# ethz-asl/laser_slam

Measured on AMD Instinct MI355X. Metric: scans_per_sec, higher is better.
Workload: dtype f32

## Files before the change

### laser_slam_amd/csrc/lsgpu_cone.hip.h

```cpp
#pragma once
#include "lsgpu_knn.hip.h"

namespace lsgpu {

constexpr int kConeGF4 = 3;
constexpr int kConePad = 16;
constexpr uint32_t kConeMaxWin = 512;

struct ConeDev {
  float ox, oy, oz;
  float z0, rs;
  float cs;
  int rows, cols;
  const float4* soa;
  const uint32_t* map;
  const uint32_t* tab;
  const float4* rowz;
};

__device__ __forceinline__ void cone_dir(float vx, float vy, float vz, float& inv_rho, float& zeta, float& pa, float& rxy,
                                         float& inv_h) {
  const float r2 = __fmaf_rn(vy, vy, vx * vx);
  inv_rho = __builtin_amdgcn_rsqf(__fmaf_rn(vz, vz, r2));
  rxy = __builtin_amdgcn_sqrtf(r2);
  zeta = vz * inv_rho;
  inv_h = __builtin_amdgcn_rcpf(fabsf(vx) + fabsf(vy));
  const float t = vy * inv_h;
  pa = vx >= 0.f ? (vy >= 0.f ? t : 4.f + t) : 2.f - t;
}

__device__ __forceinline__ uint32_t cone_clampu(float t, int hi) {
  return (uint32_t)fminf(fmaxf(t, 0.f), (float)hi);
}

__global__ __launch_bounds__(256) void k_cone_keys(const float4* __restrict__ pts, int64_t n, ConeDev c,
                                                   uint64_t* __restrict__ keys, uint32_t* __restrict__ vals) {
  const int64_t i = (int64_t)blockIdx.x * 256 + threadIdx.x;
  if (i >= n) return;
  const float4 p = pts[i];
  float inv_rho, zeta, pa, rxy, inv_h;
  cone_dir(p.x - c.ox, p.y - c.oy, p.z - c.oz, inv_rho, zeta, pa, rxy, inv_h);
  if (!(fabsf(zeta) <= 1.5f)) zeta = 0.f;
  if (!(pa >= 0.f && pa <= 4.f)) pa = 0.f;
  const uint32_t row = cone_clampu(floorf((zeta - c.z0) * c.rs), c.rows - 1);
  const uint32_t col = cone_clampu(floorf(pa * c.cs), c.cols - 1);
  keys[i] = (uint64_t)row * (uint32_t)c.cols + col;
  vals[i] = (uint32_t)i;
}

__global__ __launch_bounds__(256) void k_cone_gather(const float4* __restrict__ pts, const uint32_t* __restrict__ perm,
                                                     const uint64_t* __restrict__ keys, int64_t n, ConeDev c,
                                                     float* __restrict__ soa, uint32_t* __restrict__ map,
                                                     uint32_t* __restrict__ tab) {
  const int64_t j = (int64_t)blockIdx.x * 256 + threadIdx.x;
  const int lane = threadIdx.x & 63;
  const int64_t npad = ((n + 3) & ~(int64_t)3) + kConePad;
  const uint32_t nkeys = (uint32_t)c.rows * (uint32_t)c.cols;
  uint32_t gap_lo = 0, gap_hi = 0;
  uint32_t pos = 0;
  const bool valid = j < n;
  if (valid) {
    const uint32_t i = perm[j];
    const float4 p = pts[i];
    float* g = soa + 4 * kConeGF4 * (j >> 2) + (j & 3);
    g[0] = p.x; g[4] = p.y; g[8] = p.z; map[j] = i;
    const uint32_t key = (uint32_t)keys[j];
    gap_lo = j > 0 ? (uint32_t)keys[j - 1] + 1u : 0u;
    gap_hi = key + 1u;
    pos = (uint32_t)j;
  } else if (j < npad) {
    float* g = soa + 4 * kConeGF4 * (j >> 2) + (j & 3);
    g[0] = kPadCoord; g[4] = kPadCoord; g[8] = kPadCoord; map[j] = 0u;
    if (j == n) { gap_lo = (uint32_t)keys[n - 1] + 1u; gap_hi = nkeys + 1u; pos = (uint32_t)n; }
  }
  const uint32_t glen = gap_hi - gap_lo;
  if (glen >= 1u && glen <= 6u) {
    tab[gap_lo] = pos;
    for (uint32_t k = 1u; k < glen; ++k) tab[gap_lo + k] = pos;
// ... 431 lines not shown
```

### laser_slam_amd/csrc/lsgpu_grid.hip.h

```cpp
#pragma once
#include "lsgpu_common.hip.h"

namespace lsgpu {

struct RefStats {
  double sum[3];
  float mn[3];
  float mx[3];
  float zmn, zmx;
};

__global__ __launch_bounds__(256) void k_ref_stats(const float4* __restrict__ in, int64_t n,
                                                   RefStats* __restrict__ partials) {
  double sx = 0, sy = 0, sz = 0;
  float mnx = INFINITY, mny = INFINITY, mnz = INFINITY, mxx = -INFINITY, mxy = -INFINITY,
        mxz = -INFINITY, zmn = INFINITY, zmx = -INFINITY;
  for (int64_t i = (int64_t)blockIdx.x * 256 + threadIdx.x; i < n; i += (int64_t)gridDim.x * 256) {
    const float4 p = in[i];
    sx += p.x; sy += p.y; sz += p.z;
    mnx = fminf(mnx, p.x); mny = fminf(mny, p.y); mnz = fminf(mnz, p.z);
    mxx = fmaxf(mxx, p.x); mxy = fmaxf(mxy, p.y); mxz = fmaxf(mxz, p.z);
    const float r2 = p.x * p.x + p.y * p.y + p.z * p.z;
    if (r2 > 0.f) {
      const float zeta = p.z * __builtin_amdgcn_rsqf(r2);
// ... 68 lines not shown
      gm.mean[d] = (float)(r.sum[d] / (double)n);
      mn[d] = r.mn[d] - gm.mean[d];
      mx[d] = r.mx[d] - gm.mean[d];
      if (!isfinite(mn[d]) || !isfinite(mx[d])) gm.bad = 1;
    }
    const float ext = fmaxf(fmaxf(mx[0] - mn[0], mx[1] - mn[1]), mx[2] - mn[2]);
    int bits = 11, fine = 5;
    float h0 = cell_size_cfg > 0.f ? cell_size_cfg : 0.125f;
    while (bits < 13 && h0 * (float)((1 << bits) - 1) < ext * 1.0001f) { ++bits; --fine; }
    while (!gm.bad && h0 * (float)((1 << bits) - 1) < ext * 1.0001f) h0 *= 2.f;
    gm.ox = mn[0]; gm.oy = mn[1]; gm.oz = mn[2];
    gm.h0 = h0; gm.hf = h0 / (float)(1 << fine); gm.inv_hf = 1.0f / gm.hf; gm.fine = fine; gm.bits = bits;
    gm.zeta_lo = r.zmn; gm.zeta_hi = r.zmx;
    gm.origin_inside = 1;
    for (int d = 0; d < 3; ++d) {
      const float m = 0.1f * (r.mx[d] - r.mn[d]) + 1e-3f;
      if (!(r.mn[d] - m <= 0.f && 0.f <= r.mx[d] + m)) gm.origin_inside = 0;
    }
    if (!(r.zmn <= r.zmx)) gm.origin_inside = 0;
    *geom = gm;
  }
}

__global__ __launch_bounds__(256) void k_ref_keys(const float4* __restrict__ in, int64_t n,
                                                  const GeomDev* __restrict__ geom,
                                                  uint64_t* __restrict__ keys,
                                                  uint32_t* __restrict__ vals) {
  const int64_t i = (int64_t)blockIdx.x * 256 + threadIdx.x;
  if (i >= n) return;
  const GeomDev g = *geom;
  const float mx = g.mean[0], my = g.mean[1], mz = g.mean[2];
  const float4 p = in[i];
  const int lim = (1 << (g.bits + g.fine)) - 1;
  const int ix = fine_coord(p.x - mx, g.ox, g.inv_hf, lim);
  const int iy = fine_coord(p.y - my, g.oy, g.inv_hf, lim);
  const int iz = fine_coord(p.z - mz, g.oz, g.inv_hf, lim);
  keys[i] = morton3((uint32_t)ix, (uint32_t)iy, (uint32_t)iz);
  vals[i] = (uint32_t)i;
}

constexpr int kAngElev = 1024, kAngSect = 4096;

__device__ __forceinline__ void angular_cell(const float4& p, float inv_elev, float inv_sect, uint32_t& eb,
                                             uint32_t& sec, float& azim, float& range) {
  const float rho = sqrtf(p.x * p.x + p.y * p.y);
  const float elev = atan2f(p.z, rho);
  azim = atan2f(p.y, p.x) + 3.1415927f;
  range = sqrtf(rho * rho + p.z * p.z);
  eb = (uint32_t)fminf(fmaxf((elev + 1.5707964f) * inv_elev, 0.f), (float)(kAngElev - 1));
  sec = (uint32_t)fminf(fmaxf(azim * inv_sect, 0.f), (float)(kAngSect - 1));
}

constexpr int kDecElev = 181, kDecSect = 361, kDecCells = 65536;
__global__ __launch_bounds__(256) void k_query_ang_hist(const float4* __restrict__ in, int64_t n,
                                                        uint32_t* __restrict__ cells) {
  const int64_t i = (int64_t)blockIdx.x * 256 + threadIdx.x;
  uint32_t cell = 0xFFFFFFFFu;
  if (i < n) {
    const float4 p = in[i];
    const float elev = atan2f(p.z, sqrtf(p.x * p.x + p.y * p.y)), azim = atan2f(p.y, p.x) + 3.1415927f;
    const uint32_t eb = (uint32_t)fminf(fmaxf((elev + 1.5707964f) * 57.29578f, 0.f), (float)(kDecElev - 1));
    const uint32_t sec = (uint32_t)fminf(fmaxf(azim * 57.29578f, 0.f), (float)(kDecSect - 1));
    cell = ((eb * kDecSect + sec) * 40503u) & 0xFFFFu;
  }
  const int lane = threadIdx.x & 63;
  const uint32_t prev = (uint32_t)__shfl_up((int)cell, 1, 64);
  const bool head = lane == 0 || cell != prev;
  const unsigned long long heads = __ballot(head);
  if (head && cell != 0xFFFFFFFFu) {
    const unsigned long long later = lane == 63 ? 0ull : (heads >> (lane + 1));
    const int run = later ? __ffsll((long long)later) : 64 - lane;
    atomicAdd(&cells[cell], (uint32_t)run);
  }
}

__global__ __launch_bounds__(1024) void k_query_order(uint32_t* __restrict__ cells, int forced, float elev_deg,
                                                      float sect_deg) {
  __shared__ uint32_t occ[16], tot[16];
  uint32_t o = 0, t = 0;
  for (int i = threadIdx.x; i < kDecCells; i += 1024) { const uint32_t c = cells[i]; o += c ? 1u : 0u; t += c; }
  o = wave_sum_u32(o); t = wave_sum_u32(t);
  if ((threadIdx.x & 63) == 0) { occ[threadIdx.x >> 6] = o; tot[threadIdx.x >> 6] = t; }
  __syncthreads();
  if (threadIdx.x == 0) {
    o = 0; t = 0;
    for (int w = 0; w < 16; ++w) { o += occ[w]; t += tot[w]; }
    uint32_t* out = cells + kDecCells;
    out[0] = o; out[1] = t;
    const float m = o ? (float)t / (float)o : 54.f;
    const float f = sqrtf(54.f / fmaxf(m, 1.f));
    const float e = elev_deg > 0.f ? elev_deg : fminf(fmaxf(0.8f * f, 0.2f), 4.f);
    const float sc = sect_deg > 0.f ? sect_deg : fminf(fmaxf(0.35f * f, 0.1f), 2.f);
    const uint32_t automatic = (o < 64u && t > 4096u) ? 0u : 1u;
    out[2] = forced >= 0 ? (uint32_t)forced : automatic;
    out[3] = __float_as_uint(57.29578f / e);
    out[4] = __float_as_uint(57.29578f / sc);
  }
}

__global__ __launch_bounds__(256) void k_query_keys(const float4* __restrict__ in, int64_t n,
                                                    uint64_t* __restrict__ keys,
                                                    uint32_t* __restrict__ vals, const uint32_t* __restrict__ order_flag) {
  const int64_t i = (int64_t)blockIdx.x * 256 + threadIdx.x;
  if (i >= n) return;
  const float4 p = in[i];
  if (*order_flag == 1u) {
    uint32_t e32, s32; float azim, range;
    angular_cell(p, __uint_as_float(order_flag[1]), __uint_as_float(order_flag[2]), e32, s32, azim, range);
    const uint64_t eb = e32, sec = s32;
    const uint64_t rb = (uint64_t)fminf(fmaxf(range, 0.f), 1023.f);
    const uint64_t fine = (uint64_t)fminf(fmaxf(azim * 10430.378f, 0.f), 65535.f);
    keys[i] = (((eb * 4096ull + sec) * 1024ull + rb) << 16) | fine;
    vals[i] = (uint32_t)i;
    return;
  }
  const float lim = 65535.f, half = 32768.f;
  const uint32_t ix = (uint32_t)fminf(fmaxf(floorf(p.x * 128.f) + half, 0.f), lim);
  const uint32_t iy = (uint32_t)fminf(fmaxf(floorf(p.y * 128.f) + half, 0.f), lim);
  const uint32_t iz = (uint32_t)fminf(fmaxf(floorf(p.z * 128.f) + half, 0.f), lim);
  keys[i] = morton3(ix, iy, iz);
  vals[i] = (uint32_t)i;
}

__global__ __launch_bounds__(256) void k_ref_gather(const float4* __restrict__ in,
                                                    const float* __restrict__ nrm_in, int64_t n,
                                                    const uint32_t* __restrict__ perm,
                                                    const GeomDev* __restrict__ geom, float4* __restrict__ pts,
                                                    float4* __restrict__ nrm,
                                                    uint32_t* __restrict__ inv) {
  const float mx = geom->mean[0], my = geom->mean[1], mz = geom->mean[2];
  const int64_t j = (int64_t)blockIdx.x * 256 + threadIdx.x;
  if (j >= n) {
    if (j < n + 8) pts[j] = make_float4(3e18f, 3e18f, 3e18f, 0.f);
    return;
  }
  const uint32_t s = perm[j];
  const float4 p = in[s];
  pts[j] = make_float4(p.x - mx, p.y - my, p.z - mz, __uint_as_float(s));
  float4 nn = make_float4(0.f, 0.f, 0.f, 0.f);
  if (nrm_in) { nn.x = nrm_in[3 * (int64_t)s]; nn.y = nrm_in[3 * (int64_t)s + 1]; nn.z = nrm_in[3 * (int64_t)s + 2]; }
  nrm[j] = nn;
  inv[s] = (uint32_t)j;
}

// ... 7 lines not shown
  const float3 q = xform(T, p.x, p.y, p.z);
  out[j] = make_float4(q.x, q.y, q.z, __uint_as_float(s));
}

__global__ __launch_bounds__(256) void k_transform(const float4* __restrict__ in, int64_t n,
                                                   Mat34 T, float4* __restrict__ out) {
  const int64_t i = (int64_t)blockIdx.x * 256 + threadIdx.x;
  if (i >= n) return;
  const float4 p = in[i];
  const float3 q = xform(T, p.x, p.y, p.z);
  out[i] = make_float4(q.x, q.y, q.z, p.w);
}

__global__ __launch_bounds__(256) void k_rotate3(const float* __restrict__ in, int64_t n, Mat34 T, float* __restrict__ out) {
  const int64_t i = (int64_t)blockIdx.x * 256 + threadIdx.x;
  if (i >= n) return;
  const float x = in[3 * i], y = in[3 * i + 1], z = in[3 * i + 2];
  out[3 * i + 0] = __fmaf_rn(T.m[2], z, __fmaf_rn(T.m[1], y, T.m[0] * x));
  out[3 * i + 1] = __fmaf_rn(T.m[6], z, __fmaf_rn(T.m[5], y, T.m[4] * x));
  out[3 * i + 2] = __fmaf_rn(T.m[10], z, __fmaf_rn(T.m[9], y, T.m[8] * x));
}

__global__ __launch_bounds__(256) void k_chunk_flags(const uint64_t* __restrict__ keys, int64_t n,
                                                     const GeomDev* __restrict__ geom, uint32_t* __restrict__ flags) {
  const int64_t i = (int64_t)blockIdx.x * 256 + threadIdx.x;
  if (i >= n) return;
  const int fine = geom->fine;
  uint32_t f = ((i & (kChunkMax - 1)) == 0);
  if (i > 0 && ((keys[i] ^ keys[i - 1]) >> (3 * fine)) != 0) f = 1;
  flags[i] = f;
}

__global__ __launch_bounds__(256) void k_chunk_bounds(const uint32_t* __restrict__ flags,
                                                      const uint32_t* __restrict__ cidx, int64_t n,
                                                      uint32_t* __restrict__ bounds) {
  const int64_t i = (int64_t)blockIdx.x * 256 + threadIdx.x;
  if (i >= n) return;
  if (flags[i]) bounds[cidx[i] - 1] = (uint32_t)i;
  if (i == n - 1) bounds[cidx[i]] = (uint32_t)n;
}

__global__ __launch_bounds__(256) void k_chunk_boxes(const float4* __restrict__ pts,
                                                     const uint32_t* __restrict__ bounds,
                                                     uint32_t nchunks,
                                                     ChunkDesc* __restrict__ chunks) {
  const uint32_t c = blockIdx.x * 4u + (threadIdx.x >> 6);
  if (c >= nchunks) return;
  const int lane = threadIdx.x & 63;
// ... 132 lines not shown
```

### laser_slam_amd/csrc/lsgpu_icp.hip

```cpp
#include <cstring>
#include <cmath>
#include <cstdio>
#include <cstdlib>
#include <string>
#include <vector>
#include <chrono>
#include <functional>
#include <system_error>
#include <thread>
#include <utility>

#include <dlfcn.h>

#include <hip/hip_runtime.h>
#include <rccl/rccl.h>

#include "../../include/lsgpu_icp.h"
#include "lsgpu_grid.hip.h"
#include "lsgpu_tuning.h"
#include "lsgpu_policy.h"
#include "lsgpu_knn.hip.h"
#include "lsgpu_knn_k.hip.h"
#include "lsgpu_snf.hip.h"
#include "lsgpu_cone.hip.h"
// ... 504 lines not shown
  for (auto& bf : h->gs_k) bf.release();
  h->gs_tab.release(); h->gs_sblk.release(); h->gs_hist.release(); h->gs_cand.release(); h->gs_median.release();
  h->gs_cand_blk.release(); h->gs_cand_n.release(); h->gs_cl.release(); h->gs_err.release(); h->gs_rng.release();
  if (h->draws_pinned) (void)hipHostFree(h->draws_pinned);
  if (h->copy_done) (void)hipEventDestroy(h->copy_done);
  if (h->ref_up_done) (void)hipEventDestroy(h->ref_up_done);
  if (h->draws_done) (void)hipEventDestroy(h->draws_done);
  if (h->draws_first_done) (void)hipEventDestroy(h->draws_first_done);
  if (h->draw_stream) { (void)hipStreamSynchronize(h->draw_stream); (void)hipStreamDestroy(h->draw_stream); }
  if (h->side_done) (void)hipEventDestroy(h->side_done);
  if (h->side_stream) { (void)hipStreamSynchronize(h->side_stream); (void)hipStreamDestroy(h->side_stream); }
  if (h->copy_stream) (void)hipStreamDestroy(h->copy_stream);
  if (h->stream) (void)hipStreamDestroy(h->stream);
  delete h;
}

}


static int scan_u32(lsgpu_icp* h, const uint32_t* in, uint32_t* out, size_t n, bool inclusive = false, bool nonzero = false);

template <int ITEMS>
static void radix_pass(lsgpu_icp* h, const uint64_t* kin, const uint32_t* vin, uint64_t* kout, uint32_t* vout, int64_t n,
                       int shift, uint32_t mask, int nblocks) {
  uint32_t* bh = h->sc->sort_hist.p;
  uint32_t* dtot = bh + (size_t)256 * nblocks;
  hipLaunchKernelGGL(k_rs_hist<ITEMS>, dim3(nblocks), dim3(256), 0, h->cur, kin, n, shift, mask, bh, nblocks);
  hipLaunchKernelGGL(k_rs_scan, dim3(256), dim3(256), 0, h->cur, bh, nblocks, dtot);
  hipLaunchKernelGGL(k_rs_scatter<ITEMS>, dim3(nblocks), dim3(256), 0, h->cur, kin, vin, kout, vout, n, shift, mask,
                     bh, dtot, nblocks);
}

static int sort_pairs(lsgpu_icp* h, int64_t n, int nbits) {
  HIPC(h->sc->keys_alt.reserve(n));
  HIPC(h->sc->vals_alt.reserve(n));
  const int items_env = tuning().sort_items;
  const int items = items_env ? items_env : n >= (1 << 21) ? 16 : n >= (1 << 19) ? 8 : 4;
  const int nblocks = (int)((n + 256 * items - 1) / (256 * items));
  HIPC(h->sc->sort_hist.reserve((size_t)256 * nblocks + 256));
  const int passes = std::max(1, (nbits + 7) / 8);
  uint64_t *kin = h->sc->keys.p, *kout = h->sc->keys_alt.p;
  uint32_t *vin = h->sc->vals.p, *vout = h->sc->vals_alt.p;
  for (int p = 0; p < passes; ++p) {
    const int shift = 8 * p, width = std::max(0, std::min(8, nbits - shift));
    const uint32_t mask = (1u << width) - 1u;
    if (items == 16) radix_pass<16>(h, kin, vin, kout, vout, n, shift, mask, nblocks);
    else if (items == 8) radix_pass<8>(h, kin, vin, kout, vout, n, shift, mask, nblocks);
    else radix_pass<4>(h, kin, vin, kout, vout, n, shift, mask, nblocks);
    std::swap(kin, kout); std::swap(vin, vout);
  }
  HIPC(hipGetLastError());
  if ((passes & 1) == 0) { std::swap(h->sc->keys, h->sc->keys_alt); std::swap(h->sc->vals, h->sc->vals_alt); }
  return LSGPU_OK;
}

template <class T, class U>
static int stage_in(lsgpu_icp* h, const U* src, size_t count, DevBuf<T>& buf, const T** out) {
  if (is_device_ptr(src)) { *out = reinterpret_cast<const T*>(src); return LSGPU_OK; }
  HIPC(buf.reserve(count));
  HIPC(hipMemcpyAsync(buf.p, src, count * sizeof(T), hipMemcpyHostToDevice, h->cur));
  *out = buf.p;
  return LSGPU_OK;
}
static int stage_points(lsgpu_icp* h, const float* src, int64_t n, DevBuf<float4>& buf, const float4** out) {
  return stage_in(h, src, (size_t)n, buf, out);
}

static int ensure_loop_buffers(lsgpu_icp* h, int64_t nq) {
  HIPC(h->ids.reserve(nq));
  HIPC(h->d2.reserve(nq));
  HIPC(h->strag.reserve(nq));
  HIPC(h->hist.reserve(3 * kHistBins));
  HIPC(h->sel.reserve(4));
  HIPC(h->hist_med.reserve(3 * kHistBins)); HIPC(h->sel_med.reserve(4));
  HIPC(h->ne_partials.reserve((size_t)kNeBlocksMax * 32));
  HIPC(h->ne_gpartials.reserve((size_t)(kNeBlocksMax / kNeGroup + 1) * 32));
  HIPC(h->ne_tickets.reserve((size_t)(kNeBlocksMax / kNeGroup + 2)));
  HIPC(h->ne_out.reserve(32));
  HIPC(h->limit_dev.reserve(4));
  HIPC(h->counters.reserve(64));
  return LSGPU_OK;
}

static int prepare_queries(lsgpu_icp* h, const float* q_xyz1, int64_t nq, const Mat34& T, bool gather = true) {
  const float4* src = nullptr;
  int rc = stage_points(h, q_xyz1, nq, h->q_in, &src);
  if (rc) return rc;
  HIPC(h->sc->keys.reserve(nq));
  HIPC(h->sc->vals.reserve(nq));
  HIPC(h->rdq.reserve(nq));
  HIPC(h->prev.reserve(nq));
  HIPC(h->lb.reserve(nq));
  const int qorder = tuning().query_order;
  const float qelev = tuning().q_elev, qsect = tuning().q_sect;
  HIPC(h->ang_cells.reserve(kDecCells + 8));
  HIPC(hipMemsetAsync(h->ang_cells.p, 0, (kDecCells + 8) * sizeof(uint32_t), h->cur));
  if (qorder != 0) hipLaunchKernelGGL(k_query_ang_hist, dim3(nblk(nq)), dim3(256), 0, h->cur, src, nq, h->ang_cells.p);
  hipLaunchKernelGGL(k_query_order, dim3(1), dim3(1024), 0, h->cur, h->ang_cells.p, qorder, qelev, qsect);
  hipLaunchKernelGGL(k_query_keys, dim3(nblk(nq)), dim3(256), 0, h->cur, src, nq, h->sc->keys.p, h->sc->vals.p,
                     h->ang_cells.p + kDecCells + 2);
  rc = sort_pairs(h, nq, 48);
  if (rc) return rc;
  if (gather) {
    hipLaunchKernelGGL(k_query_gather, dim3(nblk(nq)), dim3(256), 0, h->cur, src, nq,
                       h->sc->vals_alt.p, T, h->rdq.p);
    HIPC(hipGetLastError());
  }
  h->nq = nq;
  {
    const size_t nt = (size_t)((nq + 63) / 64);
    const bool grow = nt > h->cell_tags.cap;
    HIPC(h->cell_cache.reserve(nt * 64));
    HIPC(h->cell_tags.reserve(nt));
    if (grow) HIPC(hipMemsetAsync(h->cell_tags.p, 0, h->cell_tags.cap * sizeof(ulonglong2), h->cur));
    if (++h->cache_gen == 0) h->cache_gen = 1;
  }
  h->dbg_launch_no = 0;
  return ensure_loop_buffers(h, nq);
}

static int run_select(lsgpu_icp* h, const float* d2, int n, uint32_t k, bool zero_hist, const IcpState* st,
                      bool use_comm, bool predicted, int passes = 3, float rank_ratio = 0.f, bool with_median = false);

static float matcher_max_d2(const lsgpu_icp* h) {
// ... 240 lines not shown
  const int64_t nr = h->nr;
  if (h->cfg.matcher_knn >= 2 || chain_on(h)) return false;
  if (!(tuning().cone && h->cone_origin_inside && nr >= 1024)) return false;
  return !((double)nr > 0.6 * (double)tuning().cone_max_occupancy * (double)tuning().cone_rows * (double)tuning().cone_cols);
}
static int build_cone_index(lsgpu_icp* h) {
  const int64_t nr = h->nr;
  h->cone_ok = false;
  if (!cone_wanted(h)) return LSGPU_OK;
  ConeDev c;
  std::memset(&c, 0, sizeof(c));
  c.ox = -h->mean[0]; c.oy = -h->mean[1]; c.oz = -h->mean[2];
  c.rows = tuning().cone_rows; c.cols = tuning().cone_cols;
  const float zr = std::max(h->cone_zeta_hi - h->cone_zeta_lo, 1e-3f);
  c.z0 = h->cone_zeta_lo - 1e-5f - 1e-4f * zr;
  c.rs = (float)c.rows / (zr * 1.0002f + 2e-5f);
  c.cs = (float)c.cols * 0.25f;
  const size_t npad = (((size_t)nr + 3) & ~(size_t)3) + kConePad, nkeys = (size_t)c.rows * (size_t)c.cols;
  HIPC(h->cone_soa.reserve((size_t)kConeGF4 * npad));
  HIPC(h->cone_map.reserve(npad));
  HIPC(h->cone_tab.reserve(nkeys + 1)); HIPC(h->cone_rowz.reserve((size_t)c.rows));
  HIPC(h->sc->keys.reserve(nr)); HIPC(h->sc->vals.reserve(nr));
  c.soa = reinterpret_cast<const float4*>(h->cone_soa.p); c.map = h->cone_map.p; c.tab = h->cone_tab.p; c.rowz = h->cone_rowz.p;
  hipLaunchKernelGGL(k_cone_keys, dim3(nblk(nr)), dim3(256), 0, h->cur, h->pts.p, nr, c,
                     h->sc->keys.p, h->sc->vals.p);
  int nbits = 1;
  while (((size_t)1 << nbits) < nkeys) ++nbits;
  const int rc = sort_pairs(h, nr, nbits);
  if (rc) return rc;
  HIPC(h->cone_occ.reserve(1));
  HIPC(hipMemsetAsync(h->cone_occ.p, 0, sizeof(uint32_t), h->cur));
  hipLaunchKernelGGL(k_cone_gather, dim3(nblk((int64_t)npad)), dim3(256), 0, h->cur, h->pts.p, h->sc->vals_alt.p,
                     h->sc->keys_alt.p, nr, c, h->cone_soa.p, h->cone_map.p, h->cone_tab.p);
  hipLaunchKernelGGL(k_cone_rows, dim3(c.rows), dim3(256), 0, h->cur, c, h->cone_rowz.p, h->cone_occ.p);
  HIPC(hipGetLastError());
  if (!h->cone_occ_ready) HIPC(hipEventCreateWithFlags(&h->cone_occ_ready, hipEventDisableTiming));
  if (!h->h_cone_occ) HIPC(hipHostMalloc((void**)&h->h_cone_occ, 64, hipHostMallocDefault));
  else if (hipEventSynchronize(h->cone_occ_ready) != hipSuccess) (void)hipGetLastError();
  uint32_t* ho = h->h_cone_occ;
  *ho = 0u;
  HIPC(hipMemcpyAsync(ho, h->cone_occ.p, sizeof(uint32_t), hipMemcpyDeviceToHost, h->cur));
  HIPC(hipEventRecord(h->cone_occ_ready, h->cur));
  h->cone = c;
  h->cone_ok = true;
  h->cone_decided = false;
  return LSGPU_OK;
}

static uint32_t trim_rank(int64_t n, float ratio) {
  int64_t k = (int64_t)((float)n * ratio);
  if (k >= n) k = n - 1;
  if (k < 0) k = 0;
  return (uint32_t)k;
}

extern "C" {
// ... 6 lines not shown
}

int lsgpu_icp_set_reference(lsgpu_icp* h, const float* ref_xyz1, const float* ref_normals,
                            int64_t nr) {
  if (!h) return LSGPU_BAD_ARG;
  h->err.clear();
  if (!ref_xyz1 || nr <= 0 || nr > 0x7FFFFFF0ll) { h->err = "set_reference: empty or oversize cloud"; h->nr = 0; return LSGPU_BAD_ARG; }
  HIPC(hipSetDevice(h->device));
  h->nr = 0;
  h->have_normals = ref_normals != nullptr;
  const float4* src = nullptr;
  int rc = stage_points(h, ref_xyz1, nr, h->ref_in, &src);
  if (rc) return rc;
  const float* nsrc = nullptr;
  if (ref_normals && (rc = stage_in(h, ref_normals, (size_t)3 * nr, h->nrm_in, &nsrc))) return rc;
  HIPC(h->stat_partials.reserve(kStatBlocks + 1));
  HIPC(h->geom.reserve(1));
  const int sb = std::min(kStatBlocks, nblk(nr));
  hipLaunchKernelGGL(k_ref_stats, dim3(sb), dim3(256), 0, h->stream, src, nr, h->stat_partials.p);
  hipLaunchKernelGGL(k_ref_stats_final, dim3(1), dim3(64), 0, h->stream, h->stat_partials.p, sb,
                     h->stat_partials.p + kStatBlocks, nr, h->cfg.cell_size, h->geom.p);
  HIPC(h->sc->keys.reserve(nr)); HIPC(h->sc->vals.reserve(nr));
  HIPC(h->pts.reserve(nr + 8)); HIPC(h->nrm.reserve(nr)); HIPC(h->ref_inv.reserve(nr));
  hipLaunchKernelGGL(k_ref_keys, dim3(nblk(nr)), dim3(256), 0, h->stream, src, nr, h->geom.p, h->sc->keys.p, h->sc->vals.p);
  rc = sort_pairs(h, nr, 48);
  if (rc) return rc;
  hipLaunchKernelGGL(k_ref_gather, dim3(nblk(nr + 8)), dim3(256), 0, h->stream, src, nsrc, nr,
                     h->sc->vals_alt.p, h->geom.p, h->pts.p, h->nrm.p, h->ref_inv.p);
  HIPC(h->flags.reserve(nr)); HIPC(h->cidx.reserve(nr));
  hipLaunchKernelGGL(k_chunk_flags, dim3(nblk(nr)), dim3(256), 0, h->stream, h->sc->keys_alt.p, nr, h->geom.p,
                     h->flags.p);
  rc = scan_u32(h, h->flags.p, h->cidx.p, (size_t)nr,  true);
  if (rc) return rc;
  HIPC(h->counters.reserve(64));
  HIPC(hipMemsetAsync(h->counters.p, 0, 64 * sizeof(uint32_t), h->stream));
  hipLaunchKernelGGL(k_cells_count, dim3(std::min(512, nblk(nr))), dim3(256), 0, h->stream, h->sc->keys_alt.p, nr, h->geom.p,
                     h->counters.p);
  const uint32_t* hc = h->pin->cells;
  const GeomDev* hg = &h->pin->geom;
  {
    static_assert(sizeof(GeomDev) % 4 == 0, "copied word by word");
    ToHost c{}; int used = 0;
    to_host_add(&c, &used, h->counters.p, h->pin->cells, sizeof h->pin->cells);
    to_host_add(&c, &used, h->cidx.p + (nr - 1), &h->pin->nchunks, sizeof(uint32_t));
    to_host_add(&c, &used, h->geom.p, &h->pin->geom, sizeof(GeomDev));
    hipLaunchKernelGGL(k_to_host, dim3(1), dim3(64), 0, h->stream, c);
    HIPC(hipGetLastError());
  }
  if (h->hook_before_ref_sync) {
    rc = h->hook_before_ref_sync();
    if (rc) return rc;
  }
  HIPC(hipStreamSynchronize(h->stream));
  if (hg->bad) { h->err = "set_reference: non-finite coordinates"; return LSGPU_BAD_ARG; }
  for (int d = 0; d < 3; ++d) h->mean[d] = hg->mean[d];
  const int bits = hg->bits, fine = hg->fine;
  const float h0 = hg->h0;
  GridDev g;
// ... 2064 lines not shown
```

### laser_slam_amd/csrc/lsgpu_sort.hip.h

```cpp
#pragma once
#include <hip/hip_runtime.h>
#include <stdint.h>

namespace lsgpu {

__device__ __forceinline__ uint32_t wave_scan_incl_u32(uint32_t v, int lane) {
#pragma unroll
  for (int o = 1; o < 64; o <<= 1) {
    const uint32_t t = (uint32_t)__shfl_up((int)v, o, 64);
    if (lane >= o) v += t;
  }
  return v;
}

template <int ITEMS>
__global__ __launch_bounds__(256) void k_rs_hist(const uint64_t* __restrict__ keys, int64_t n, int shift,
                                                 uint32_t mask, uint32_t* __restrict__ blockhist, int nblocks) {
  __shared__ uint32_t hist[256];
  hist[threadIdx.x] = 0u;
  __syncthreads();
  const int lane = threadIdx.x & 63, w = threadIdx.x >> 6;
  const int64_t base = (int64_t)blockIdx.x * (256 * ITEMS) + (int64_t)w * (64 * ITEMS) + lane;
  uint64_t k[ITEMS];
#pragma unroll
  for (int i = 0; i < ITEMS; ++i) {
    const int64_t idx = base + i * 64;
    k[i] = idx < n ? keys[idx] : 0ull;
  }
#pragma unroll
  for (int i = 0; i < ITEMS; ++i)
    if (base + i * 64 < n) atomicAdd(&hist[(uint32_t)(k[i] >> shift) & mask], 1u);
  __syncthreads();
  blockhist[(size_t)threadIdx.x * nblocks + blockIdx.x] = hist[threadIdx.x];
}

// ... 118 lines not shown
```

### laser_slam_amd/csrc/lsgpu_tuning.h

```cpp

#pragma once
#include <cstdio>
#include <cstdlib>
#include <cstring>

extern char** environ;

namespace lsgpu {

struct Tuning {
  int query_order = -1;
  float q_elev = 0.f, q_sect = 0.f;
  float gap = 0.002f;
  int chunk_budget = 512, chunk_budget_wide = 1024;
  int wide_iters = 3;
  float route_r = 0.02f;
  int route_chunks = 1024;
  int route_heavy_max = 1024;
  int route_dense = 512;
  bool predict_select = true, commit_select = true, comm_commit = true, seed_cap = true;
  int sel_amb_cap = 256;
  bool two_pass_select = true;
  bool short_last_group = true;
  bool fused_select = true;
  bool lazy_need = true;
  bool lane_split = true;
  bool lookahead = true;
  bool index_rest = true;
  bool side_stream = true;
  int front_guess = 2048;
  int sort_items = 0;
  bool ssn_sort_levels = false;
  int ssn_root = 0;
  int ne_blocks = 256;
  bool split_update = false;
  double comm_timeout_ms = 30000.0;
  int knn_dbg = 0;
  bool cone = true;
  bool cone_probe = true;
  int cone_rows = 128, cone_cols = 8192, cone_from = 2;
  float cone_max_occupancy = 7.0f;
  float cone_heavy_steps = 1024.f;
  float cone_heavy_share = 0.07f;
};

namespace tuning_detail {
inline bool flag(const char* name) { return getenv(name) != nullptr; }
inline double number(const char* name, double def, double lo, double hi) {
  const char* e = getenv(name);
  if (!e) return def;
  char* end = nullptr;
  const double v = strtod(e, &end);
  if (end == e || *end != '\0' || !(v >= lo && v <= hi)) {
    fprintf(stderr, "liblsgpu_icp: %s=%s is not a number in [%g, %g]; using the default %g\n", name, e, lo, hi, def);
// ... 14 lines not shown
  t.route_chunks = (int)number("LSGPU_ROUTE_CHUNKS", 1024, 1, 1 << 30);
  t.route_heavy_max = (int)number("LSGPU_ROUTE_HEAVY_MAX", 1024, -1, 1 << 30);
  t.route_dense = (int)number("LSGPU_ROUTE_DENSE", 512, 1, 1 << 30);
  t.split_update = flag("LSGPU_SPLIT_UPDATE");
  t.predict_select = !flag("LSGPU_NO_PREDICT") && !t.split_update;
  t.commit_select = !flag("LSGPU_NO_COMMIT");
  t.fused_select = !flag("LSGPU_NO_FUSED_SELECT");
  t.short_last_group = !flag("LSGPU_FULL_GROUPS");
  t.two_pass_select = !flag("LSGPU_THREE_PASS_SELECT");
  t.sel_amb_cap = (int)number("LSGPU_SEL_AMB_CAP", 256, 0, 256);
  t.comm_commit = !flag("LSGPU_NO_COMM_COMMIT");
  t.seed_cap = !flag("LSGPU_NO_SEED_CAP");
  t.lazy_need = !flag("LSGPU_NO_LAZY");
  t.lane_split = !flag("LSGPU_NO_SPLIT");
  t.side_stream = !flag("LSGPU_NO_SIDE_STREAM");
  t.lookahead = !flag("LSGPU_NO_LOOKAHEAD");
  t.index_rest = !flag("LSGPU_NO_INDEX_REST");
  t.front_guess = (int)number("LSGPU_FRONT_GUESS", 2048, 0, 8192);
  t.sort_items = (int)number("LSGPU_SORT_ITEMS", 0, 0, 16);
  if (t.sort_items != 0 && t.sort_items != 4 && t.sort_items != 8 && t.sort_items != 16) {
    fprintf(stderr, "liblsgpu_icp: LSGPU_SORT_ITEMS must be 4, 8 or 16; choosing by size\n");
    t.sort_items = 0;
  }
  t.ssn_sort_levels = flag("LSGPU_SSN_SORT_LEVELS");
  t.ssn_root = (int)number("LSGPU_SSN_ROOT", 0, 0, 8192);
  if (t.ssn_root != 0 && t.ssn_root != 2048 && t.ssn_root != 4096 && t.ssn_root != 8192) {
    fprintf(stderr, "liblsgpu_icp: LSGPU_SSN_ROOT must be 2048, 4096 or 8192; choosing by size\n");
    t.ssn_root = 0;
  }
  t.ne_blocks = (int)number("LSGPU_NE_BLOCKS", 256, 64, 2048);
  t.comm_timeout_ms = number("LSGPU_COMM_TIMEOUT_MS", 30000, 1, 1e9);
  t.knn_dbg = (int)number("LSGPU_KNN_DBG", 0, 0, 1 << 20);
  t.cone = !flag("LSGPU_NO_CONE");
  t.cone_probe = !flag("LSGPU_NO_CONE_PROBE");
  t.cone_from = (int)number("LSGPU_CONE_FROM", 2, 1, 1 << 20);
  t.cone_max_occupancy = (float)number("LSGPU_CONE_MAX_OCC", 7.0, 0.0, 1e9);
  t.cone_heavy_steps = (float)number("LSGPU_CONE_HEAVY_STEPS", 1024.0, 0.0, 1e9);
  t.cone_heavy_share = (float)number("LSGPU_CONE_HEAVY_SHARE", 0.07, 0.0, 2.0);
  t.cone_rows = (int)number("LSGPU_CONE_ROWS", 128, 8, 1024);
  t.cone_cols = (int)number("LSGPU_CONE_COLS", 8192, 64, 65536) & ~3;
  static const char* known[] = {"LSGPU_QUERY_ORDER", "LSGPU_Q_ELEV", "LSGPU_Q_SECT", "LSGPU_GAP", "LSGPU_BUDGET", "LSGPU_BUDGET_WIDE", "LSGPU_WIDE_ITERS",
                                "LSGPU_ROUTE_R", "LSGPU_ROUTE_CHUNKS", "LSGPU_ROUTE_HEAVY_MAX", "LSGPU_ROUTE_DENSE", "LSGPU_SPLIT_UPDATE", "LSGPU_NO_PREDICT", "LSGPU_NO_COMMIT",
                                "LSGPU_NO_COMM_COMMIT", "LSGPU_NO_SEED_CAP", "LSGPU_NO_LAZY", "LSGPU_NO_SPLIT", "LSGPU_NO_SIDE_STREAM", "LSGPU_NO_LOOKAHEAD", "LSGPU_NO_INDEX_REST", "LSGPU_CELLS_SPLIT", "LSGPU_NO_FUSED_SELECT", "LSGPU_FULL_GROUPS", "LSGPU_THREE_PASS_SELECT", "LSGPU_SEL_AMB_CAP", "LSGPU_FRONT_GUESS",
                                "LSGPU_SORT_ITEMS", "LSGPU_SSN_ROOT", "LSGPU_SSN_SORT_LEVELS",
                                "LSGPU_NE_BLOCKS", "LSGPU_COMM_TIMEOUT_MS", "LSGPU_KNN_DBG", "LSGPU_NO_CONE", "LSGPU_NO_CONE_PROBE", "LSGPU_CONE_ROWS", "LSGPU_CONE_COLS", "LSGPU_CONE_FROM", "LSGPU_CONE_MAX_OCC", "LSGPU_CONE_HEAVY_STEPS", "LSGPU_CONE_HEAVY_SHARE",
                                "LSGPU_SO", "LSGPU_STATS_SO", "LSGPU_BATCH_POOLS", "LSGPU_BATCH_UNIQ", "LSGPU_GS_DEBUG", "LSGPU_GOLDEN_DIR", "LSGPU_SEQ_PERTURB", "LSGPU_SEQ_POSES", "LSGPU_TEST_INPUT_FILTERS",
                                nullptr};
  for (char** e = environ; e && *e; ++e) {
    if (strncmp(*e, "LSGPU_", 6) != 0) continue;
    const char* eq = strchr(*e, '=');
    const size_t len = eq ? (size_t)(eq - *e) : strlen(*e);
    bool ok = false;
    for (const char** k = known; *k; ++k) ok = ok || (strlen(*k) == len && strncmp(*k, *e, len) == 0);
    if (!ok) fprintf(stderr, "liblsgpu_icp: unknown switch %.*s ignored (see csrc/lsgpu_tuning.h)\n", (int)len, *e);
  }
  return t;
}
}

inline const Tuning& tuning() {
  static const Tuning t = tuning_detail::read();
  return t;
}

}
```

Measured before the change: 251.1.

## Fuse first radix histogram into key kernels and fold memsets into kernels

The key-generation kernels for query, reference and cone sorts now also build the first radix pass's per-block histogram, so the separate histogram kernel for pass 0 is skipped. Several hipMemsetAsync calls (angular cells, cone occupancy, counters) are folded into existing kernels, which clear the buffers themselves. This removes a few launches and one full read of the keys per sort. In exchange the key kernels do shared-memory atomics and use the sort's tile layout, and correctness depends on the in-kernel clears running before the buffers are next used.

```diff
diff --git a/laser_slam_amd/csrc/lsgpu_cone.hip.h b/laser_slam_amd/csrc/lsgpu_cone.hip.h
--- a/laser_slam_amd/csrc/lsgpu_cone.hip.h
+++ b/laser_slam_amd/csrc/lsgpu_cone.hip.h
@@ -1,5 +1,6 @@
 #pragma once
 #include "lsgpu_knn.hip.h"
+#include "lsgpu_sort.hip.h"
 
 namespace lsgpu {
 
@@ -33,27 +34,36 @@
   return (uint32_t)fminf(fmaxf(t, 0.f), (float)hi);
 }
 
-__global__ __launch_bounds__(256) void k_cone_keys(const float4* __restrict__ pts, int64_t n, ConeDev c,
-                                                   uint64_t* __restrict__ keys, uint32_t* __restrict__ vals) {
-  const int64_t i = (int64_t)blockIdx.x * 256 + threadIdx.x;
-  if (i >= n) return;
-  const float4 p = pts[i];
+__device__ __forceinline__ uint64_t cone_key(const float4 p, const ConeDev& c) {
   float inv_rho, zeta, pa, rxy, inv_h;
   cone_dir(p.x - c.ox, p.y - c.oy, p.z - c.oz, inv_rho, zeta, pa, rxy, inv_h);
   if (!(fabsf(zeta) <= 1.5f)) zeta = 0.f;
   if (!(pa >= 0.f && pa <= 4.f)) pa = 0.f;
   const uint32_t row = cone_clampu(floorf((zeta - c.z0) * c.rs), c.rows - 1);
   const uint32_t col = cone_clampu(floorf(pa * c.cs), c.cols - 1);
-  keys[i] = (uint64_t)row * (uint32_t)c.cols + col;
+  return (uint64_t)row * (uint32_t)c.cols + col;
+}
+__global__ __launch_bounds__(256) void k_cone_keys(const float4* __restrict__ pts, int64_t n, ConeDev c,
+                                                   uint64_t* __restrict__ keys, uint32_t* __restrict__ vals) {
+  const int64_t i = (int64_t)blockIdx.x * 256 + threadIdx.x;
+  if (i >= n) return;
+  keys[i] = cone_key(pts[i], c);
   vals[i] = (uint32_t)i;
+}
+template <int ITEMS>
+__global__ __launch_bounds__(256) void k_cone_keys_hist(const float4* __restrict__ pts, int64_t n, ConeDev c,
+                                                        uint64_t* __restrict__ keys, uint32_t* __restrict__ vals, uint32_t mask,
+                                                        uint32_t* __restrict__ blockhist, int nblocks) {
+  rs_keys_tile<ITEMS>(n, mask, keys, vals, blockhist, nblocks, [&](int64_t i) { return cone_key(pts[i], c); });
 }
 
 __global__ __launch_bounds__(256) void k_cone_gather(const float4* __restrict__ pts, const uint32_t* __restrict__ perm,
                                                      const uint64_t* __restrict__ keys, int64_t n, ConeDev c,
                                                      float* __restrict__ soa, uint32_t* __restrict__ map,
-                                                     uint32_t* __restrict__ tab) {
+                                                     uint32_t* __restrict__ tab, uint32_t* __restrict__ occ_clear) {
   const int64_t j = (int64_t)blockIdx.x * 256 + threadIdx.x;
   const int lane = threadIdx.x & 63;
+  if (occ_clear && j == 0) *occ_clear = 0u;
   const int64_t npad = ((n + 3) & ~(int64_t)3) + kConePad;
   const uint32_t nkeys = (uint32_t)c.rows * (uint32_t)c.cols;
   uint32_t gap_lo = 0, gap_hi = 0;
diff --git a/laser_slam_amd/csrc/lsgpu_grid.hip.h b/laser_slam_amd/csrc/lsgpu_grid.hip.h
--- a/laser_slam_amd/csrc/lsgpu_grid.hip.h
+++ b/laser_slam_amd/csrc/lsgpu_grid.hip.h
@@ -1,5 +1,6 @@
 #pragma once
 #include "lsgpu_common.hip.h"
+#include "lsgpu_sort.hip.h"
 
 namespace lsgpu {
 
@@ -114,6 +115,13 @@
   }
 }
 
+__device__ __forceinline__ uint64_t ref_key(const float4 p, const GeomDev& g) {
+  const int lim = (1 << (g.bits + g.fine)) - 1;
+  const int ix = fine_coord(p.x - g.mean[0], g.ox, g.inv_hf, lim);
+  const int iy = fine_coord(p.y - g.mean[1], g.oy, g.inv_hf, lim);
+  const int iz = fine_coord(p.z - g.mean[2], g.oz, g.inv_hf, lim);
+  return morton3((uint32_t)ix, (uint32_t)iy, (uint32_t)iz);
+}
 __global__ __launch_bounds__(256) void k_ref_keys(const float4* __restrict__ in, int64_t n,
                                                   const GeomDev* __restrict__ geom,
                                                   uint64_t* __restrict__ keys,
@@ -121,14 +129,15 @@
   const int64_t i = (int64_t)blockIdx.x * 256 + threadIdx.x;
   if (i >= n) return;
   const GeomDev g = *geom;
-  const float mx = g.mean[0], my = g.mean[1], mz = g.mean[2];
-  const float4 p = in[i];
-  const int lim = (1 << (g.bits + g.fine)) - 1;
-  const int ix = fine_coord(p.x - mx, g.ox, g.inv_hf, lim);
-  const int iy = fine_coord(p.y - my, g.oy, g.inv_hf, lim);
-  const int iz = fine_coord(p.z - mz, g.oz, g.inv_hf, lim);
-  keys[i] = morton3((uint32_t)ix, (uint32_t)iy, (uint32_t)iz);
+  keys[i] = ref_key(in[i], g);
   vals[i] = (uint32_t)i;
+}
+template <int ITEMS>
+__global__ __launch_bounds__(256) void k_ref_keys_hist(const float4* __restrict__ in, int64_t n, const GeomDev* __restrict__ geom,
+                                                       uint64_t* __restrict__ keys, uint32_t* __restrict__ vals, uint32_t mask,
+                                                       uint32_t* __restrict__ blockhist, int nblocks) {
+  const GeomDev g = *geom;
+  rs_keys_tile<ITEMS>(n, mask, keys, vals, blockhist, nblocks, [&](int64_t i) { return ref_key(in[i], g); });
 }
 
 constexpr int kAngElev = 1024, kAngSect = 4096;
@@ -167,10 +176,13 @@
 }
 
 __global__ __launch_bounds__(1024) void k_query_order(uint32_t* __restrict__ cells, int forced, float elev_deg,
-                                                      float sect_deg) {
+                                                      float sect_deg, int rearm) {
   __shared__ uint32_t occ[16], tot[16];
   uint32_t o = 0, t = 0;
-  for (int i = threadIdx.x; i < kDecCells; i += 1024) { const uint32_t c = cells[i]; o += c ? 1u : 0u; t += c; }
+  for (int i = threadIdx.x; i < kDecCells; i += 1024) {
+    const uint32_t c = cells[i]; o += c ? 1u : 0u; t += c;
+    if (rearm && c) cells[i] = 0u;
+  }
   o = wave_sum_u32(o); t = wave_sum_u32(t);
   if ((threadIdx.x & 63) == 0) { occ[threadIdx.x >> 6] = o; tot[threadIdx.x >> 6] = t; }
   __syncthreads();
@@ -190,28 +202,34 @@
   }
 }
 
-__global__ __launch_bounds__(256) void k_query_keys(const float4* __restrict__ in, int64_t n,
-                                                    uint64_t* __restrict__ keys,
-                                                    uint32_t* __restrict__ vals, const uint32_t* __restrict__ order_flag) {
-  const int64_t i = (int64_t)blockIdx.x * 256 + threadIdx.x;
-  if (i >= n) return;
-  const float4 p = in[i];
+__device__ __forceinline__ uint64_t query_key(const float4 p, const uint32_t* __restrict__ order_flag) {
   if (*order_flag == 1u) {
     uint32_t e32, s32; float azim, range;
     angular_cell(p, __uint_as_float(order_flag[1]), __uint_as_float(order_flag[2]), e32, s32, azim, range);
     const uint64_t eb = e32, sec = s32;
     const uint64_t rb = (uint64_t)fminf(fmaxf(range, 0.f), 1023.f);
     const uint64_t fine = (uint64_t)fminf(fmaxf(azim * 10430.378f, 0.f), 65535.f);
-    keys[i] = (((eb * 4096ull + sec) * 1024ull + rb) << 16) | fine;
-    vals[i] = (uint32_t)i;
-    return;
+    return (((eb * 4096ull + sec) * 1024ull + rb) << 16) | fine;
   }
   const float lim = 65535.f, half = 32768.f;
   const uint32_t ix = (uint32_t)fminf(fmaxf(floorf(p.x * 128.f) + half, 0.f), lim);
   const uint32_t iy = (uint32_t)fminf(fmaxf(floorf(p.y * 128.f) + half, 0.f), lim);
   const uint32_t iz = (uint32_t)fminf(fmaxf(floorf(p.z * 128.f) + half, 0.f), lim);
-  keys[i] = morton3(ix, iy, iz);
+  return morton3(ix, iy, iz);
+}
+__global__ __launch_bounds__(256) void k_query_keys(const float4* __restrict__ in, int64_t n,
+                                                    uint64_t* __restrict__ keys,
+                                                    uint32_t* __restrict__ vals, const uint32_t* __restrict__ order_flag) {
+  const int64_t i = (int64_t)blockIdx.x * 256 + threadIdx.x;
+  if (i >= n) return;
+  keys[i] = query_key(in[i], order_flag);
   vals[i] = (uint32_t)i;
+}
+template <int ITEMS>
+__global__ __launch_bounds__(256) void k_query_keys_hist(const float4* __restrict__ in, int64_t n, uint64_t* __restrict__ keys,
+                                                         uint32_t* __restrict__ vals, const uint32_t* __restrict__ order_flag,
+                                                         uint32_t mask, uint32_t* __restrict__ blockhist, int nblocks) {
+  rs_keys_tile<ITEMS>(n, mask, keys, vals, blockhist, nblocks, [&](int64_t i) { return query_key(in[i], order_flag); });
 }
 
 __global__ __launch_bounds__(256) void k_ref_gather(const float4* __restrict__ in,
@@ -265,8 +283,10 @@
 }
 
 __global__ __launch_bounds__(256) void k_chunk_flags(const uint64_t* __restrict__ keys, int64_t n,
-                                                     const GeomDev* __restrict__ geom, uint32_t* __restrict__ flags) {
-  const int64_t i = (int64_t)blockIdx.x * 256 + threadIdx.x;
+                                                     const GeomDev* __restrict__ geom, uint32_t* __restrict__ flags,
+                                                     uint32_t* __restrict__ clear64) {
+  const int64_t i = (int64_t)blockIdx.x * 256 + threadIdx.x;
+  if (clear64 && blockIdx.x == 0 && threadIdx.x < 64) clear64[threadIdx.x] = 0u;
   if (i >= n) return;
   const int fine = geom->fine;
   uint32_t f = ((i & (kChunkMax - 1)) == 0);
diff --git a/laser_slam_amd/csrc/lsgpu_icp.hip b/laser_slam_amd/csrc/lsgpu_icp.hip
--- a/laser_slam_amd/csrc/lsgpu_icp.hip
+++ b/laser_slam_amd/csrc/lsgpu_icp.hip
@@ -550,31 +550,49 @@
 
 template <int ITEMS>
 static void radix_pass(lsgpu_icp* h, const uint64_t* kin, const uint32_t* vin, uint64_t* kout, uint32_t* vout, int64_t n,
-                       int shift, uint32_t mask, int nblocks) {
+                       int shift, uint32_t mask, int nblocks, bool hist_ready) {
   uint32_t* bh = h->sc->sort_hist.p;
   uint32_t* dtot = bh + (size_t)256 * nblocks;
-  hipLaunchKernelGGL(k_rs_hist<ITEMS>, dim3(nblocks), dim3(256), 0, h->cur, kin, n, shift, mask, bh, nblocks);
+  if (!hist_ready) hipLaunchKernelGGL(k_rs_hist<ITEMS>, dim3(nblocks), dim3(256), 0, h->cur, kin, n, shift, mask, bh, nblocks);
   hipLaunchKernelGGL(k_rs_scan, dim3(256), dim3(256), 0, h->cur, bh, nblocks, dtot);
   hipLaunchKernelGGL(k_rs_scatter<ITEMS>, dim3(nblocks), dim3(256), 0, h->cur, kin, vin, kout, vout, n, shift, mask,
                      bh, dtot, nblocks);
 }
 
-static int sort_pairs(lsgpu_icp* h, int64_t n, int nbits) {
+struct SortTiles { int items, nblocks; };
+static SortTiles sort_tiles(int64_t n) {
+  SortTiles t;
+  t.items = rs_items(n, tuning().sort_items);
+  t.nblocks = rs_blocks(n, t.items);
+  return t;
+}
+static int sort_reserve_hist(lsgpu_icp* h, const SortTiles& t) {
+  HIPC(h->sc->sort_hist.reserve((size_t)256 * t.nblocks + 256));
+  return LSGPU_OK;
+}
+#define LSGPU_LAUNCH_KEYS_HIST(KERNEL, tiles, ...)                                                                          \
+  do {                                                                                                                      \
+    if ((tiles).items == 16) hipLaunchKernelGGL(KERNEL<16>, dim3((tiles).nblocks), dim3(256), 0, h->cur, __VA_ARGS__);      \
+    else if ((tiles).items == 8) hipLaunchKernelGGL(KERNEL<8>, dim3((tiles).nblocks), dim3(256), 0, h->cur, __VA_ARGS__);   \
+    else hipLaunchKernelGGL(KERNEL<4>, dim3((tiles).nblocks), dim3(256), 0, h->cur, __VA_ARGS__);                           \
+  } while (0)
+
+static int sort_pairs(lsgpu_icp* h, int64_t n, int nbits, bool hist0_ready = false) {
   HIPC(h->sc->keys_alt.reserve(n));
   HIPC(h->sc->vals_alt.reserve(n));
-  const int items_env = tuning().sort_items;
-  const int items = items_env ? items_env : n >= (1 << 21) ? 16 : n >= (1 << 19) ? 8 : 4;
-  const int nblocks = (int)((n + 256 * items - 1) / (256 * items));
-  HIPC(h->sc->sort_hist.reserve((size_t)256 * nblocks + 256));
+  const SortTiles tl = sort_tiles(n);
+  const int items = tl.items, nblocks = tl.nblocks;
+  if (!hist0_ready) { const int rc = sort_reserve_hist(h, tl); if (rc) return rc; }
   const int passes = std::max(1, (nbits + 7) / 8);
   uint64_t *kin = h->sc->keys.p, *kout = h->sc->keys_alt.p;
   uint32_t *vin = h->sc->vals.p, *vout = h->sc->vals_alt.p;
   for (int p = 0; p < passes; ++p) {
-    const int shift = 8 * p, width = std::max(0, std::min(8, nbits - shift));
-    const uint32_t mask = (1u << width) - 1u;
-    if (items == 16) radix_pass<16>(h, kin, vin, kout, vout, n, shift, mask, nblocks);
-    else if (items == 8) radix_pass<8>(h, kin, vin, kout, vout, n, shift, mask, nblocks);
-    else radix_pass<4>(h, kin, vin, kout, vout, n, shift, mask, nblocks);
+    const int shift = 8 * p;
+    const uint32_t mask = rs_mask(nbits, p);
+    const bool ready = hist0_ready && p == 0;
+    if (items == 16) radix_pass<16>(h, kin, vin, kout, vout, n, shift, mask, nblocks, ready);
+    else if (items == 8) radix_pass<8>(h, kin, vin, kout, vout, n, shift, mask, nblocks, ready);
+    else radix_pass<4>(h, kin, vin, kout, vout, n, shift, mask, nblocks, ready);
     std::swap(kin, kout); std::swap(vin, vout);
   }
   HIPC(hipGetLastError());
@@ -621,13 +639,24 @@
   HIPC(h->lb.reserve(nq));
   const int qorder = tuning().query_order;
   const float qelev = tuning().q_elev, qsect = tuning().q_sect;
+  const bool rearm = tuning().fold_fills;
+  const bool fresh_cells = h->ang_cells.cap == 0;
   HIPC(h->ang_cells.reserve(kDecCells + 8));
-  HIPC(hipMemsetAsync(h->ang_cells.p, 0, (kDecCells + 8) * sizeof(uint32_t), h->cur));
+  if (fresh_cells || !rearm) HIPC(hipMemsetAsync(h->ang_cells.p, 0, (kDecCells + 8) * sizeof(uint32_t), h->cur));
   if (qorder != 0) hipLaunchKernelGGL(k_query_ang_hist, dim3(nblk(nq)), dim3(256), 0, h->cur, src, nq, h->ang_cells.p);
-  hipLaunchKernelGGL(k_query_order, dim3(1), dim3(1024), 0, h->cur, h->ang_cells.p, qorder, qelev, qsect);
-  hipLaunchKernelGGL(k_query_keys, dim3(nblk(nq)), dim3(256), 0, h->cur, src, nq, h->sc->keys.p, h->sc->vals.p,
-                     h->ang_cells.p + kDecCells + 2);
-  rc = sort_pairs(h, nq, 48);
+  hipLaunchKernelGGL(k_query_order, dim3(1), dim3(1024), 0, h->cur, h->ang_cells.p, qorder, qelev, qsect, rearm ? 1 : 0);
+  const bool key_hist = tuning().key_hist;
+  if (key_hist) {
+    const SortTiles tl = sort_tiles(nq);
+    rc = sort_reserve_hist(h, tl);
+    if (rc) return rc;
+    LSGPU_LAUNCH_KEYS_HIST(k_query_keys_hist, tl, src, nq, h->sc->keys.p, h->sc->vals.p, (const uint32_t*)(h->ang_cells.p + kDecCells + 2),
+                           rs_mask(48, 0), h->sc->sort_hist.p, tl.nblocks);
+  } else {
+    hipLaunchKernelGGL(k_query_keys, dim3(nblk(nq)), dim3(256), 0, h->cur, src, nq, h->sc->keys.p, h->sc->vals.p,
+                       h->ang_cells.p + kDecCells + 2);
+  }
+  rc = sort_pairs(h, nq, 48, key_hist);
   if (rc) return rc;
   if (gather) {
     hipLaunchKernelGGL(k_query_gather, dim3(nblk(nq)), dim3(256), 0, h->cur, src, nq,
@@ -914,16 +943,26 @@
   HIPC(h->cone_tab.reserve(nkeys + 1)); HIPC(h->cone_rowz.reserve((size_t)c.rows));
   HIPC(h->sc->keys.reserve(nr)); HIPC(h->sc->vals.reserve(nr));
   c.soa = reinterpret_cast<const float4*>(h->cone_soa.p); c.map = h->cone_map.p; c.tab = h->cone_tab.p; c.rowz = h->cone_rowz.p;
-  hipLaunchKernelGGL(k_cone_keys, dim3(nblk(nr)), dim3(256), 0, h->cur, h->pts.p, nr, c,
-                     h->sc->keys.p, h->sc->vals.p);
   int nbits = 1;
   while (((size_t)1 << nbits) < nkeys) ++nbits;
-  const int rc = sort_pairs(h, nr, nbits);
+  const bool key_hist = tuning().key_hist;
+  if (key_hist) {
+    const SortTiles tl = sort_tiles(nr);
+    const int rc0 = sort_reserve_hist(h, tl);
+    if (rc0) return rc0;
+    LSGPU_LAUNCH_KEYS_HIST(k_cone_keys_hist, tl, (const float4*)h->pts.p, nr, c, h->sc->keys.p, h->sc->vals.p, rs_mask(nbits, 0),
+                           h->sc->sort_hist.p, tl.nblocks);
+  } else {
+    hipLaunchKernelGGL(k_cone_keys, dim3(nblk(nr)), dim3(256), 0, h->cur, h->pts.p, nr, c,
+                       h->sc->keys.p, h->sc->vals.p);
+  }
+  const int rc = sort_pairs(h, nr, nbits, key_hist);
   if (rc) return rc;
   HIPC(h->cone_occ.reserve(1));
-  HIPC(hipMemsetAsync(h->cone_occ.p, 0, sizeof(uint32_t), h->cur));
+  const bool fold = tuning().fold_fills;
+  if (!fold) HIPC(hipMemsetAsync(h->cone_occ.p, 0, sizeof(uint32_t), h->cur));
   hipLaunchKernelGGL(k_cone_gather, dim3(nblk((int64_t)npad)), dim3(256), 0, h->cur, h->pts.p, h->sc->vals_alt.p,
-                     h->sc->keys_alt.p, nr, c, h->cone_soa.p, h->cone_map.p, h->cone_tab.p);
+                     h->sc->keys_alt.p, nr, c, h->cone_soa.p, h->cone_map.p, h->cone_tab.p, fold ? h->cone_occ.p : (uint32_t*)nullptr);
   hipLaunchKernelGGL(k_cone_rows, dim3(c.rows), dim3(256), 0, h->cur, c, h->cone_rowz.p, h->cone_occ.p);
   HIPC(hipGetLastError());
   if (!h->cone_occ_ready) HIPC(hipEventCreateWithFlags(&h->cone_occ_ready, hipEventDisableTiming));
@@ -976,18 +1015,28 @@
                      h->stat_partials.p + kStatBlocks, nr, h->cfg.cell_size, h->geom.p);
   HIPC(h->sc->keys.reserve(nr)); HIPC(h->sc->vals.reserve(nr));
   HIPC(h->pts.reserve(nr + 8)); HIPC(h->nrm.reserve(nr)); HIPC(h->ref_inv.reserve(nr));
-  hipLaunchKernelGGL(k_ref_keys, dim3(nblk(nr)), dim3(256), 0, h->stream, src, nr, h->geom.p, h->sc->keys.p, h->sc->vals.p);
-  rc = sort_pairs(h, nr, 48);
+  const bool key_hist = tuning().key_hist;
+  if (key_hist) {
+    const SortTiles tl = sort_tiles(nr);
+    rc = sort_reserve_hist(h, tl);
+    if (rc) return rc;
+    LSGPU_LAUNCH_KEYS_HIST(k_ref_keys_hist, tl, src, nr, (const GeomDev*)h->geom.p, h->sc->keys.p, h->sc->vals.p, rs_mask(48, 0),
+                           h->sc->sort_hist.p, tl.nblocks);
+  } else {
+    hipLaunchKernelGGL(k_ref_keys, dim3(nblk(nr)), dim3(256), 0, h->stream, src, nr, h->geom.p, h->sc->keys.p, h->sc->vals.p);
+  }
+  rc = sort_pairs(h, nr, 48, key_hist);
   if (rc) return rc;
   hipLaunchKernelGGL(k_ref_gather, dim3(nblk(nr + 8)), dim3(256), 0, h->stream, src, nsrc, nr,
                      h->sc->vals_alt.p, h->geom.p, h->pts.p, h->nrm.p, h->ref_inv.p);
   HIPC(h->flags.reserve(nr)); HIPC(h->cidx.reserve(nr));
+  HIPC(h->counters.reserve(64));
+  const bool fold = tuning().fold_fills;
   hipLaunchKernelGGL(k_chunk_flags, dim3(nblk(nr)), dim3(256), 0, h->stream, h->sc->keys_alt.p, nr, h->geom.p,
-                     h->flags.p);
+                     h->flags.p, fold ? h->counters.p : (uint32_t*)nullptr);
   rc = scan_u32(h, h->flags.p, h->cidx.p, (size_t)nr,  true);
   if (rc) return rc;
-  HIPC(h->counters.reserve(64));
-  HIPC(hipMemsetAsync(h->counters.p, 0, 64 * sizeof(uint32_t), h->stream));
+  if (!fold) HIPC(hipMemsetAsync(h->counters.p, 0, 64 * sizeof(uint32_t), h->stream));
   hipLaunchKernelGGL(k_cells_count, dim3(std::min(512, nblk(nr))), dim3(256), 0, h->stream, h->sc->keys_alt.p, nr, h->geom.p,
                      h->counters.p);
   const uint32_t* hc = h->pin->cells;
diff --git a/laser_slam_amd/csrc/lsgpu_sort.hip.h b/laser_slam_amd/csrc/lsgpu_sort.hip.h
--- a/laser_slam_amd/csrc/lsgpu_sort.hip.h
+++ b/laser_slam_amd/csrc/lsgpu_sort.hip.h
@@ -11,6 +11,35 @@
     if (lane >= o) v += t;
   }
   return v;
+}
+
+inline int rs_items(int64_t n, int forced) { return forced ? forced : n >= (1 << 21) ? 16 : n >= (1 << 19) ? 8 : 4; }
+inline int rs_blocks(int64_t n, int items) { return (int)((n + 256 * (int64_t)items - 1) / (256 * (int64_t)items)); }
+inline uint32_t rs_mask(int nbits, int pass) {
+  const int width = nbits - 8 * pass;
+  return (1u << (width < 0 ? 0 : width > 8 ? 8 : width)) - 1u;
+}
+
+template <int ITEMS, class KeyOf>
+__device__ __forceinline__ void rs_keys_tile(int64_t n, uint32_t mask, uint64_t* __restrict__ keys, uint32_t* __restrict__ vals,
+                                             uint32_t* __restrict__ blockhist, int nblocks, KeyOf key_of) {
+  __shared__ uint32_t hist[256];
+  hist[threadIdx.x] = 0u;
+  __syncthreads();
+  const int lane = threadIdx.x & 63, w = threadIdx.x >> 6;
+  const int64_t base = (int64_t)blockIdx.x * (256 * ITEMS) + (int64_t)w * (64 * ITEMS) + lane;
+#pragma unroll
+  for (int i = 0; i < ITEMS; ++i) {
+    const int64_t idx = base + i * 64;
+    if (idx < n) {
+      const uint64_t k = key_of(idx);
+      keys[idx] = k;
+      vals[idx] = (uint32_t)idx;
+      atomicAdd(&hist[(uint32_t)k & mask], 1u);
+    }
+  }
+  __syncthreads();
+  blockhist[(size_t)threadIdx.x * nblocks + blockIdx.x] = hist[threadIdx.x];
 }
 
 template <int ITEMS>
diff --git a/laser_slam_amd/csrc/lsgpu_tuning.h b/laser_slam_amd/csrc/lsgpu_tuning.h
--- a/laser_slam_amd/csrc/lsgpu_tuning.h
+++ b/laser_slam_amd/csrc/lsgpu_tuning.h
@@ -30,6 +30,8 @@
   bool side_stream = true;
   int front_guess = 2048;
   int sort_items = 0;
+  bool key_hist = true;
+  bool fold_fills = true;
   bool ssn_sort_levels = false;
   int ssn_root = 0;
   int ne_blocks = 256;
@@ -90,6 +92,8 @@
     fprintf(stderr, "liblsgpu_icp: LSGPU_SORT_ITEMS must be 4, 8 or 16; choosing by size\n");
     t.sort_items = 0;
   }
+  t.key_hist = !flag("LSGPU_NO_KEY_HIST");
+  t.fold_fills = !flag("LSGPU_NO_FOLD_FILLS");
   t.ssn_sort_levels = flag("LSGPU_SSN_SORT_LEVELS");
   t.ssn_root = (int)number("LSGPU_SSN_ROOT", 0, 0, 8192);
   if (t.ssn_root != 0 && t.ssn_root != 2048 && t.ssn_root != 4096 && t.ssn_root != 8192) {
@@ -110,7 +114,7 @@
   static const char* known[] = {"LSGPU_QUERY_ORDER", "LSGPU_Q_ELEV", "LSGPU_Q_SECT", "LSGPU_GAP", "LSGPU_BUDGET", "LSGPU_BUDGET_WIDE", "LSGPU_WIDE_ITERS",
                                 "LSGPU_ROUTE_R", "LSGPU_ROUTE_CHUNKS", "LSGPU_ROUTE_HEAVY_MAX", "LSGPU_ROUTE_DENSE", "LSGPU_SPLIT_UPDATE", "LSGPU_NO_PREDICT", "LSGPU_NO_COMMIT",
                                 "LSGPU_NO_COMM_COMMIT", "LSGPU_NO_SEED_CAP", "LSGPU_NO_LAZY", "LSGPU_NO_SPLIT", "LSGPU_NO_SIDE_STREAM", "LSGPU_NO_LOOKAHEAD", "LSGPU_NO_INDEX_REST", "LSGPU_CELLS_SPLIT", "LSGPU_NO_FUSED_SELECT", "LSGPU_FULL_GROUPS", "LSGPU_THREE_PASS_SELECT", "LSGPU_SEL_AMB_CAP", "LSGPU_FRONT_GUESS",
-                                "LSGPU_SORT_ITEMS", "LSGPU_SSN_ROOT", "LSGPU_SSN_SORT_LEVELS",
+                                "LSGPU_SORT_ITEMS", "LSGPU_NO_KEY_HIST", "LSGPU_NO_FOLD_FILLS", "LSGPU_SSN_ROOT", "LSGPU_SSN_SORT_LEVELS",
                                 "LSGPU_NE_BLOCKS", "LSGPU_COMM_TIMEOUT_MS", "LSGPU_KNN_DBG", "LSGPU_NO_CONE", "LSGPU_NO_CONE_PROBE", "LSGPU_CONE_ROWS", "LSGPU_CONE_COLS", "LSGPU_CONE_FROM", "LSGPU_CONE_MAX_OCC", "LSGPU_CONE_HEAVY_STEPS", "LSGPU_CONE_HEAVY_SHARE",
                                 "LSGPU_SO", "LSGPU_STATS_SO", "LSGPU_BATCH_POOLS", "LSGPU_BATCH_UNIQ", "LSGPU_GS_DEBUG", "LSGPU_GOLDEN_DIR", "LSGPU_SEQ_PERTURB", "LSGPU_SEQ_POSES", "LSGPU_TEST_INPUT_FILTERS",
                                 nullptr};
```

Result: no change. 249.5 (-0.7%).
